# NoSuchThingAsRandom/EpidemicSimulator

Hardware: AMD Instinct MI355X
Metric: citizen-timesteps/sec (higher is better)
Workload: dtype u32 citizen word; u32 uniform vs ceil(q*2^32) (reference: f64 uniform; tolerance 2^-32 per draw); 1 GPU; uk64m: 64000000 citizens, 290000 Output Areas, 10 seeds, steps 1..667 of 5000, interventions on; seed=1592598545

## Files before the change

### epidemicsimulator_amd/csrc/esim_kernels_chunk.h

```cpp
#pragma once
#define BF_WIN 1024
__device__ __forceinline__ void block_scan_1024(uint32_t *v, uint32_t *wtmp)
{
    const uint32_t tid = threadIdx.x, lane = tid & 63u, wv = tid >> 6;
    uint32_t x = v[tid];
#pragma unroll
    for (int o = 1; o < 64; o <<= 1) { const uint32_t y = __shfl_up(x, o, 64); if (lane >= (uint32_t)o) x += y; }
    if (lane == 63u) wtmp[wv] = x;
    __syncthreads();
    if (tid == 0) { uint32_t a = 0; for (uint32_t w = 0; w < FIN_TPB / 64; ++w) { const uint32_t y = wtmp[w]; wtmp[w] = a; a += y; } }
    __syncthreads();
    v[tid] = x + wtmp[wv];
    __syncthreads();
}

__device__ __forceinline__ void future_body(const Dev &d, uint32_t max_ahead, uint32_t limit_t, uint32_t *win, uint32_t *wtmp)
{
    Ctrl *ctrl = d.ctrl;
    const uint32_t t0 = ld(&ctrl->t), tid = threadIdx.x;
    const uint32_t n_ahead = t0 > limit_t ? 0u : (limit_t - t0 + 1u < max_ahead ? limit_t - t0 + 1u : max_ahead);
    const int et = (int)d.exposed_time, it = (int)d.infected_time;
    const int base_idx = (int)(t0 + TE_BIAS) - et - 1 - it;
    { const int k = base_idx + (int)tid; win[tid] = (k >= 0 && k < (int)TE_SLOTS) ? ld(&d.hist[k]) : 0u; }
    __syncthreads();
// ... 926 lines not shown
}

struct ChunkShared {
    Decision dec[FREE_MAX];
    uint64_t thr[512];
};
struct RouteShared {
    uint32_t s_key[CHUNK_ROUTE_MAX];
    uint16_t s_bus[CHUNK_ROUTE_MAX];
    uint8_t s_inf[CHUNK_ROUTE_MAX];
    uint32_t s_cnt[CHUNK_ROUTE_MAX + 1];
};
#define SLOT_STEPS 4u
struct WaveScratch { uint32_t rounds; uint32_t cnt[FREE_MAX]; uint32_t sch[FREE_MAX]; uint32_t mem_id[64]; uint32_t mem_w[64]; uint4 desc[2u * (FREE_MAX / SLOT_STEPS + 1u)]; };

__device__ __forceinline__ void member_pairs(const Dev &d, Ctrl *ctrl, const ChunkShared &sm, WaveScratch &ws, const uint32_t *idx,
                                             uint32_t lo, uint32_t p_lo, uint32_t p_hi, uint32_t lane, uint32_t kind, uint32_t S, uint32_t t0 WORK_ARG,
                                             bool have_pre = false, uint32_t pre_m = 0u, uint32_t pre_w = 0u, uint32_t pre_base = 0u)
{
    const uint64_t seed = ((uint64_t)d.seed_hi << 32) | d.seed_lo;
    const uint32_t m_first = p_lo / S, m_last = (p_hi - 1u) / S;
    for (uint32_t mb = m_first; mb <= m_last; mb += 64u) {
        __builtin_amdgcn_wave_barrier();
        if (mb + lane <= m_last) {
            WORK_ADD(WK_MEMBERS, 1); WORK_ADD(WK_MEMBERS_IDX, idx ? 1 : 0);
            if (have_pre && mb == pre_base) { ws.mem_id[lane] = pre_m; ws.mem_w[lane] = pre_w; }
            else {
                const uint32_t m = idx ? idx[lo + mb + lane] : lo + mb + lane;
                ws.mem_id[lane] = m;
                ws.mem_w[lane] = d.cit[m];
            }
        }
        __builtin_amdgcn_wave_barrier();
        const uint32_t q_lo = max(p_lo, mb * S), q_hi = min(p_hi, (mb + 64u) * S);
#ifdef ESIM_WAVE_PROFILE
        if (lane == 0) ws.rounds += (q_hi - q_lo + 63u) / 64u;
#endif
        for (uint32_t p = q_lo + lane; p < q_hi; p += 64u) {
            const uint32_t um = p / S, si = p - um * S;
            const uint32_t m = ws.mem_id[um - mb], w = ws.mem_w[um - mb];
            const uint32_t te = CW_TE(w);
            WORK_ADD(WK_PAIRS, 1);
            if (te >= TE_RECOVERED && te != TE_SUSCEPTIBLE) continue;
            const uint4 dsc = ws.desc[2u * si];
            const uint32_t cnt23 = ws.desc[2u * si + 1u].x;
            const int jb = (int)(dsc.x & 127u) - 3;
            const uint32_t mk = (dsc.x >> 8) & 15u, atw = (dsc.x >> 12) & 15u, everywhere = (dsc.x >> 16) & 15u;
            const uint32_t vrel = CW_VAX_REL(w);
            const int js = (int)te + (((w & ~CW_KEEP) & ((1u << CW_TE_SHIFT) - 1u)) ? 1 : 0) - (int)(t0 + TE_BIAS);
            const int lim = min(js, vrel == CW_VAX_NONE ? (int)FREE_MAX : (int)vrel + 1) - jb;
            const uint32_t early = lim <= 0 ? 0u : lim >= (int)SLOT_STEPS ? 15u : (1u << lim) - 1u;
            const bool same = w & FL_SAME_AREA;
            const uint32_t here = kind == 0u ? (((w & FL_HAS_WORK) && !same) ? ~atw : 15u) : (same ? 15u : atw);
            const uint32_t act = mk & early & here;
            if (!act) continue;
            WORK_ADD(WK_PAIRS_ACTIVE, 1);
            const uint32_t nn = kind == 2u ? dsc.z : dsc.y;
            const uint32_t row = (w & FL_MASK_COMPLIANT) ? 0u : everywhere;
            uint64_t thr[SLOT_STEPS];
#pragma unroll
            for (uint32_t h = 0; h < SLOT_STEPS; ++h) thr[h] = sm.thr[(((row >> h) & 1u) << 8) + ((nn >> (8u * h)) & 255u)];
            const uint32_t gid = d.id_base + m;
            const uint32_t s_blk = (uint32_t)((int)t0 + jb) + (uint32_t)__builtin_ctz(act);
            uint32_t hit = 0u;
            if (kind == 2u) {
                const uint32_t cnt[SLOT_STEPS] = { dsc.w & 0xFFFFu, dsc.w >> 16, cnt23 & 0xFFFFu, cnt23 >> 16 };
                uint32_t kmax = 0u;
#pragma unroll
                for (uint32_t h = 0; h < SLOT_STEPS; ++h) if ((act >> h) & 1u) kmax = max(kmax, cnt[h]);
                const uint32_t first_act = act & (0u - act);
#ifdef ESIM_COUNT_WORK
                for (uint32_t h = 0; h < SLOT_STEPS; ++h) if ((act >> h) & 1u) WORK_ADD(WK_DRAWS, cnt[h]);
#endif
                for (uint32_t k = 0; k < kmax && !(hit & first_act); ++k) {
                    WORK_ADD(WK_BLOCKS, 1);
                    const philox_out o = esim_draw_block(seed, gid, s_blk, ESIM_SLOT_ROOM0 + k);
                    const uint32_t wd[SLOT_STEPS] = { o.w0, o.w1, o.w2, o.w3 };
#pragma unroll
                    for (uint32_t h = 0; h < SLOT_STEPS; ++h) if (((act >> h) & 1u) && k < cnt[h] && (uint64_t)wd[h] < thr[h]) hit |= 1u << h;
                }
            } else {
                WORK_ADD(WK_BLOCKS, 1); WORK_ADD(WK_DRAWS, __popc(act));
                const philox_out o = esim_draw_block(seed, gid, s_blk, kind == 0u ? ESIM_SLOT_HOME : ESIM_SLOT_WORK);
                const uint32_t wd[SLOT_STEPS] = { o.w0, o.w1, o.w2, o.w3 };
#pragma unroll
                for (uint32_t h = 0; h < SLOT_STEPS; ++h) if ((uint64_t)wd[h] < thr[h]) hit |= 1u << h;
                hit &= act;
            }
            if (hit) { WORK_ADD(WK_HITS, 1); expose_min(d, ctrl, m, w, (uint32_t)((int)t0 + jb) + (uint32_t)__builtin_ctz(hit), 0u); }
        }
    }
}

__device__ __forceinline__ uint32_t m96_nibble(const M96 &m, int p)
{
    if (p < 0) return (uint32_t)(m.lo << (-p)) & 15u;
    if (p >= 64) return p >= 96 ? 0u : (m.hi >> (p - 64)) & 15u;
    return (uint32_t)((m.lo >> p) | (p > 60 ? (unsigned long long)m.hi << (64 - p) : 0ull)) & 15u;
}

__device__ __forceinline__ uint32_t item_steps_regs(uint32_t c0, uint32_t c1, uint32_t lane, WaveScratch &ws, uint32_t t0, const M96 &AW, const M96 &EV)
{
    ws.cnt[lane] = c0;
    if (lane < FREE_MAX - 64u) ws.cnt[64u + lane] = c1;
// ... 28 lines not shown
__device__ __forceinline__ uint32_t fetch_slot(const Dev &d, uint32_t slot, uint32_t lane);
__device__ __forceinline__ void item_counts(const Dev &d, uint32_t x, uint32_t slot, uint32_t lane, uint32_t n, const M96 &AW,
                                            const M96 &BUS, uint32_t &c0, uint32_t &c1);
__device__ __forceinline__ void school_counts(const Dev &d, uint32_t s_sch, uint32_t lane, uint32_t n, const Decision &q0, const Decision &q1, WaveScratch &ws)
{
    uint32_t c0 = 0u, c1 = 0u;
    if (s_sch != 0xFFFFFFFFu) {
        if (lane < n) c0 = d.vec[(size_t)s_sch * FREE_MAX + lane];
        if (64u + lane < n) c1 = d.vec[(size_t)s_sch * FREE_MAX + 64u + lane];
    }
    ws.sch[lane] = c0;
    if (lane < FREE_MAX - 64u) ws.sch[64u + lane] = c1;
}

struct UnitSrc { uint32_t slot, link, own; };
__device__ __forceinline__ void list_or_units(const Dev &d, Ctrl *ctrl, const ChunkShared &sm, WaveScratch &ws, const uint32_t *idx,
                                              uint32_t lo, uint32_t hi, const UnitSrc &src, uint32_t lane, uint32_t kind, uint32_t S, uint32_t t0 WORK_ARG,
                                              bool have_pre = false, uint32_t pre_m = 0u, uint32_t pre_w = 0u)
{
    const uint32_t pairs = (hi - lo) * S;
    if (pairs == 0) return;
    if (pairs <= UNIT_INLINE) { member_pairs(d, ctrl, sm, ws, idx, lo, 0u, pairs, lane, kind, S, t0 WORK_PASS, have_pre, pre_m, pre_w); return; }
    const uint32_t n_units = (pairs + UNIT_PAIRS - 1u) / UNIT_PAIRS;
    const uint32_t r = ((blockIdx.x * TPB + threadIdx.x) >> 6) & (SUBQ - 1u);
    uint32_t start = 0;
    if (lane == 0) start = atomicAdd(&d.hot[(HOT_UNITS + r) * HOT_STRIDE], n_units);
    start = __shfl(start, 0, 64);
    UnitRec *q = d.units + (size_t)r * d.unit_qcap;
    if (start + n_units > d.unit_qcap) {
        for (uint32_t i = lane; i < n_units && start + i < d.unit_qcap; i += 64u) q[start + i].code = UNIT_NOOP;
        member_pairs(d, ctrl, sm, ws, idx, lo, 0u, pairs, lane, kind, S, t0 WORK_PASS, have_pre, pre_m, pre_w);
        return;
    }
    for (uint32_t i = lane; i < n_units; i += 64u) {
        const uint32_t p_lo = i * UNIT_PAIRS;
        q[start + i] = UnitRec{ src.slot, kind == 2u ? src.link : 0xFFFFFFFFu, lo, hi - lo, (kind << 30) | p_lo, src.own, p_lo / S, 0u };
    }
}

struct ItemFetch { uint32_t slot, id, a_lo, a_hi, b_lo, b_hi, aux, link, c0, c1; };
__device__ __forceinline__ uint32_t fetch_item(const Dev &d, uint32_t v, uint32_t lane)
{
    uint32_t x = 0u;
    if (lane < 8u) x = reinterpret_cast<const uint32_t *>(d.item_rec)[(size_t)v * 8u + lane];
    else if (lane == LANE_HSLOT) x = d.hitems[v];
    return x;
// ... 36 lines not shown
    if (f.slot < d.hcap) {
        item_counts(d, x, f.slot, lane, n, AW, BUS, f.c0, f.c1);
        iv_count(FX(x, 7), lane, AW, BUS, f.c0, f.c1);
    }
    return f;
}

__device__ __forceinline__ bool item_ok(const Dev &d, const ItemFetch &it)
{
    if (it.slot >= d.hcap) return false;
    if (it.id < d.n_bld) return it.a_lo <= it.a_hi && it.a_hi <= d.n && it.b_lo <= it.b_hi && it.b_hi <= d.n_wrk_idx;
    if (it.id < d.n_bld + d.n_room) return it.a_lo <= it.a_hi && it.a_hi <= d.n_room_idx && (it.link == 0xFFFFFFFFu || it.link < d.hcap);
    return true;
}
#define PAIR_SPREAD 1237u
__device__ __forceinline__ void route_pair_small(const Dev &d, Ctrl *ctrl, const ChunkShared &sm, uint32_t off, uint32_t sz, uint32_t j, uint32_t t0, uint32_t lane WORK_ARG)
{
    const uint64_t seed = ((uint64_t)d.seed_hi << 32) | d.seed_lo;
    const uint32_t s = t0 + j, mask = sm.dec[j].mask;
    uint32_t c = 0, w = 0, key = 0;
    bool inf = false;
    WORK_ADD(WK_ROUTE_PAIRS, lane == 0 ? 1 : 0); WORK_ADD(WK_RIDERS, lane < sz ? 1 : 0);
    bool can = false;
    if (lane < sz) {
        c = d.route_riders[off + lane];
        w = d.cit[c];
        inf = status_in_chunk(d, w, t0, j) == ESIM_INFECTED;
        const uint32_t te = CW_TE(w);
        can = !(w <= CW_MAKE(s + TE_BIAS, CW_BUS_EXPOSED | (w & CW_KEEP)) || (te >= TE_RECOVERED && te != TE_SUSCEPTIBLE) || j > CW_VAX_REL(w));
    }
    if (!__any(inf) || !__any(can)) return;
    uint32_t rank = 0;
    if (sz > d.bus_capacity) {
        if (lane < sz) key = philox4x32_10(d.id_base + c, s, ESIM_SLOT_BUS_ORDER, 0u, d.seed_lo, d.seed_hi).w0;
        for (uint32_t i = 0; i < sz; ++i) {
            const uint32_t ki = (uint32_t)__builtin_amdgcn_readlane((int)key, (int)i);
            rank += ki < key || (ki == key && i < lane);
        }
    }
    const uint32_t bus = rank / d.bus_capacity;
    const unsigned long long inf_m = __ballot(inf);
    uint32_t k = 0;
    const uint32_t n_bus = (sz + d.bus_capacity - 1u) / d.bus_capacity;
    for (uint32_t b = 0; b < n_bus; ++b) {
        const unsigned long long on_b = __ballot(lane < sz && bus == b);
        if (bus == b) k = (uint32_t)__popcll(on_b & inf_m);
    }
    if (lane < sz && k && can) {
        const uint32_t row = (!(w & FL_MASK_COMPLIANT) && mask == ESIM_MASK_EVERYWHERE) ? 1u : 0u;
        WORK_ADD(WK_BUS_DRAWS, 1);
        if (esim_u32(seed, d.id_base + c, s, ESIM_SLOT_BUS) < sm.thr[row * 256u + (k & 255u)]) { WORK_ADD(WK_HITS, 1); expose_min(d, ctrl, c, w, s, CW_BUS_EXPOSED); }
    }
}

template <uint32_t NT>
__device__ __forceinline__ void route_pair_big(const Dev &d, Ctrl *ctrl, const ChunkShared &sm, RouteShared &rs, uint32_t code, uint32_t t0, uint32_t n WORK_ARG)
{
    const uint64_t seed = ((uint64_t)d.seed_hi << 32) | d.seed_lo;
    const uint32_t r = code >> 7, j = code & 127u;
    if (r >= d.n_routes || j >= n) { if (threadIdx.x == 0) ctrl->error = (uint32_t)(-ESIM_ERANGE); return; }
    const uint32_t off = d.route_off[r], sz = d.route_off[r + 1] - off;
    if (sz > CHUNK_ROUTE_MAX) { if (threadIdx.x == 0) ctrl->error = (uint32_t)(-ESIM_ERANGE); return; }
    const uint32_t s = t0 + j, mask = sm.dec[j].mask;
    WORK_ADD(WK_ROUTE_PAIRS, threadIdx.x == 0 ? 1 : 0);
    int loc_inf = 0, loc_can = 0;
    for (uint32_t i = threadIdx.x; i < sz; i += NT) {
        const uint32_t c = d.route_riders[off + i];
// ... 19 lines not shown
    }
    __syncthreads();
    for (uint32_t i = threadIdx.x; i < sz; i += NT) {
        const uint32_t k = rs.s_cnt[rs.s_bus[i]];
        if (!k) continue;
        const uint32_t c = d.route_riders[off + i];
        const uint32_t w = d.cit[c], te = CW_TE(w);
        if (w <= CW_MAKE(s + TE_BIAS, CW_BUS_EXPOSED | (w & CW_KEEP)) || (te >= TE_RECOVERED && te != TE_SUSCEPTIBLE) || j > CW_VAX_REL(w)) continue;
        const uint32_t row = (!(w & FL_MASK_COMPLIANT) && mask == ESIM_MASK_EVERYWHERE) ? 1u : 0u;
        WORK_ADD(WK_BUS_DRAWS, 1);
        if (esim_u32(seed, d.id_base + c, s, ESIM_SLOT_BUS) < sm.thr[row * 256u + (k & 255u)]) { WORK_ADD(WK_HITS, 1); expose_min(d, ctrl, c, w, s, CW_BUS_EXPOSED); }
    }
    __syncthreads();
}

__global__ __launch_bounds__(TPB) void k_chunk_draw(Dev d, uint32_t n_mw)
{
    __shared__ ChunkShared sm;
    __shared__ WaveScratch wsc[TPB / 64];
    Ctrl *ctrl = d.ctrl;
    const uint32_t t0 = ctrl->chunk_t0, n = ctrl->chunk_ok;
    if (!ctrl->chunk_parallel || n == 0u) return;
    const uint32_t lane = threadIdx.x & 63u;
    const uint32_t wave = (blockIdx.x * TPB + threadIdx.x) >> 6, n_waves = (gridDim.x * TPB) >> 6;
    const uint32_t pt0 = PROF_NOW();
    WORK_TALLY;
    uint32_t p_items = 0u, p_item_max = 0u;
    const uint32_t per_wave = ld(&ctrl->items_per_wave);
    if ((unsigned long long)per_wave * n_mw > d.items_cap || n_waves % n_mw != 0u) return;
    const uint32_t G = n_waves / n_mw;
    const uint32_t T = d.used_pref[n_mw];
    const uint32_t coarse = d.used_pref[min(64u * lane, n_mw)];
    const uint32_t Tq = T / n_waves, Tr = T % n_waves;
    const uint32_t d_lo = Tq * wave + (uint32_t)(((unsigned long long)Tr * wave) / n_waves), d_hi = Tq * (wave + 1u) + (uint32_t)(((unsigned long long)Tr * (wave + 1u)) / n_waves);
// ... 20 lines not shown
    uint32_t code_l = 0u, off_l = 0u, sz_l = 0u;
    bool have = false;
    {
        const uint32_t k = lane * G + w_rep;
        if (k < K) {
            const uint32_t src = (w_base + n_mw - (uint32_t)(((unsigned long long)k * PAIR_SPREAD) % n_mw)) % n_mw;
            code_l = d.route_pairs[(size_t)src * K + k];
            have = k < d.pair_cnt[src] && (code_l >> 7) < d.n_routes && (code_l & 127u) < n;
        }
    }
    for (uint32_t i = threadIdx.x; i < n; i += TPB) sm.dec[i] = d.dec[i];
    for (uint32_t i = threadIdx.x; i < 512u; i += TPB) sm.thr[i] = d.thr[i];
    __syncthreads();
    const uint32_t route_base = d.n_bld + d.n_room;
    WaveScratch &ws = wsc[threadIdx.x >> 6];
    const Decision q0 = lane < n ? sm.dec[lane] : Decision{ 0u, 0u, 0u, 0u };
    const Decision q1 = 64u + lane < n ? sm.dec[64u + lane] : Decision{ 0u, 0u, 0u, 0u };
    M96 AW, BUS;
    schedule_masks(lane, n, q0, q1, AW, BUS);
    const M96 EV = { __ballot(lane < n && q0.mask == ESIM_MASK_EVERYWHERE), (uint32_t)__ballot(64u + lane < n && q1.mask == ESIM_MASK_EVERYWHERE) };
    if (d_lo < d_hi) sl_cur = fetch_slot(d, FX(id_cur, LANE_HSLOT), lane);
    if (have) { const uint32_t r = code_l >> 7; off_l = d.route_off[r]; sz_l = d.route_off[r + 1] - off_l; }
#ifdef ESIM_WAVE_PROFILE
    if (lane == 0) ws.rounds = 0u;
#endif
    uint32_t pst[5] = { 0u, 0u, 0u, 0u, 0u };
    const uint32_t pt1 = PROF_NOW();
    for (uint32_t v = d_lo; v < d_hi; ++v) {
        const uint32_t x = merge_fetch(id_cur, sl_cur, lane);
        id_cur = id_nxt;
// ... 8 lines not shown
        pst[0] += pi0 - pq0;
        (void)pi0; ++p_items; WORK_ADD(WK_ITEMS, lane == 0 ? 1 : 0);
        if (it.id < d.n_bld) {
            if (it.aux == ESIM_SCHOOL) continue;
            const uint32_t n_res = it.a_hi - it.a_lo, n_wrk = it.b_hi - it.b_lo;
            uint32_t rm = 0u, wm = 0u, rw = 0u, ww = 0u;
            if (lane < n_res) rm = d.res_idx ? d.res_idx[it.a_lo + lane] : it.a_lo + lane;
            if (lane < n_wrk) wm = d.wrk_idx[it.b_lo + lane];
            if (lane < n_res) rw = d.cit[rm];
            if (lane < n_wrk) ww = d.cit[wm];
            const uint32_t pq1 = PROF_NOW();
            const uint32_t S = item_steps_regs(it.c0, it.c1, lane, ws, t0, AW, EV);
            __builtin_amdgcn_wave_barrier();
            const uint32_t pq2 = PROF_NOW();
            const UnitSrc src = { it.slot, it.link, FX(x, 7) };
            list_or_units(d, ctrl, sm, ws, d.res_idx, it.a_lo, it.a_hi, src, lane, 0u, S, t0 WORK_PASS, true, rm, rw);
            const uint32_t pq3 = PROF_NOW();
            list_or_units(d, ctrl, sm, ws, d.wrk_idx, it.b_lo, it.b_hi, src, lane, 1u, S, t0 WORK_PASS, true, wm, ww);
            const uint32_t pq4 = PROF_NOW();
            pst[1] += pq1 - pi0; pst[2] += pq2 - pq1; pst[3] += pq3 - pq2; pst[4] += pq4 - pq3;
        } else {
            const uint32_t n_mem = it.a_hi - it.a_lo;
            uint32_t mm = 0u, mw = 0u;
            if (lane < n_mem) mm = d.room_idx[it.a_lo + lane];
            school_counts(d, it.link, lane, n, q0, q1, ws);
            if (lane < n_mem) mw = d.cit[mm];
            const uint32_t S = item_steps_regs(it.c0, it.c1, lane, ws, t0, AW, EV);
            __builtin_amdgcn_wave_barrier();
            const UnitSrc src = { it.slot, it.link, FX(x, 7) };
            list_or_units(d, ctrl, sm, ws, d.room_idx, it.a_lo, it.a_hi, src, lane, 2u, S, t0 WORK_PASS, true, mm, mw);
        }
        __builtin_amdgcn_wave_barrier();
        { const uint32_t dt = PROF_NOW() - pi0; p_item_max = dt > p_item_max ? dt : p_item_max; }
    }
    const uint32_t pt2 = PROF_NOW();
    for (uint32_t k0 = 0; k0 * G < K; k0 += 64u) {
        if (k0) {
            const uint32_t kk = (k0 + lane) * G + w_rep;
            have = false;
            if (kk < K) {
                const uint32_t src = (w_base + n_mw - (uint32_t)(((unsigned long long)kk * PAIR_SPREAD) % n_mw)) % n_mw;
                code_l = d.route_pairs[(size_t)src * K + kk];
                have = kk < d.pair_cnt[src] && (code_l >> 7) < d.n_routes && (code_l & 127u) < n;
            }
            if (have) { const uint32_t r = code_l >> 7; off_l = d.route_off[r]; sz_l = d.route_off[r + 1] - off_l; }
        }
        unsigned long long todo = __ballot(have);
        while (todo) {
            const int src_lane = __ffsll((long long)todo) - 1;
            todo &= todo - 1ull;
            const uint32_t code = __shfl(code_l, src_lane, 64), off = __shfl(off_l, src_lane, 64), sz = __shfl(sz_l, src_lane, 64);
            route_pair_small(d, ctrl, sm, off, sz, code & 127u, t0, lane WORK_PASS);
        }
    }
    WORK_FLUSH(d);
    const uint32_t pt3 = PROF_NOW();
#ifndef ESIM_PROFILE_UNITS
    PROF_PUT(d, 0, pt0); PROF_PUT(d, 1, pt1); PROF_PUT(d, 2, pt2); PROF_PUT(d, 3, pt3);
    PROF_PUT(d, 4, p_items); PROF_PUT(d, 5, p_item_max); PROF_PUT(d, 6, wsc[threadIdx.x >> 6].rounds);
    PROF_PUT(d, 11, pst[0]); PROF_PUT(d, 12, pst[1]); PROF_PUT(d, 13, pst[2]); PROF_PUT(d, 14, pst[3]); PROF_PUT(d, 15, pst[4]);
#endif
    (void)pst;
    (void)pt0; (void)pt1; (void)pt2; (void)pt3; (void)p_items; (void)p_item_max;
}

__global__ __launch_bounds__(TPB) void k_chunk_units(Dev d)
{
    __shared__ ChunkShared sm;
    __shared__ WaveScratch wsc[TPB / 64];
// ... 2 lines not shown
    const uint32_t t0 = ctrl->chunk_t0, n = ctrl->chunk_ok;
    if (!ctrl->chunk_parallel || n == 0u) return;
    const uint32_t lane = threadIdx.x & 63u;
    const uint32_t wave = (blockIdx.x * TPB + threadIdx.x) >> 6, n_waves = (gridDim.x * TPB) >> 6;
    const uint32_t pu0 = PROF_NOW();
    WORK_TALLY;
    uint32_t pu_n = 0u, pu_max = 0u, pu_it = 0u;
    const uint32_t qr = wave & (SUBQ - 1u), first = wave / SUBQ, step = n_waves / SUBQ;
    const uint32_t n_units = step ? min(ld(&d.hot[(HOT_UNITS + qr) * HOT_STRIDE]), d.unit_qcap) : 0u;
    const uint32_t n_pairs = min(ld(&d.hot[HOT_BIGPAIRS * HOT_STRIDE]), d.big_pairs_cap);
    if (__syncthreads_or(first < n_units) == 0 && n_pairs == 0u) return;
    for (uint32_t i = threadIdx.x; i < n; i += TPB) sm.dec[i] = d.dec[i];
    for (uint32_t i = threadIdx.x; i < 512u; i += TPB) sm.thr[i] = d.thr[i];
    __syncthreads();
    WaveScratch &ws = wsc[threadIdx.x >> 6];
    const uint32_t *q_words = reinterpret_cast<const uint32_t *>(d.units + (size_t)qr * d.unit_qcap);
    const Decision q0 = lane < n ? sm.dec[lane] : Decision{ 0u, 0u, 0u, 0u };
    const Decision q1 = 64u + lane < n ? sm.dec[64u + lane] : Decision{ 0u, 0u, 0u, 0u };
    M96 AW, BUS;
    schedule_masks(lane, n, q0, q1, AW, BUS);
    const M96 EV = { __ballot(lane < n && q0.mask == ESIM_MASK_EVERYWHERE), (uint32_t)__ballot(64u + lane < n && q1.mask == ESIM_MASK_EVERYWHERE) };
    auto unit_words = [&](uint32_t q) -> uint32_t { return lane < 8u ? q_words[(size_t)q * 8u + lane] : 0u; };
    auto member_id = [&](uint32_t u) -> uint32_t {
        const uint32_t code = FX(u, 4), kind = code >> 30, lo = FX(u, 2), n_mem = FX(u, 3), mf = FX(u, 6);
        if (code == UNIT_NOOP || mf + lane >= n_mem) return 0u;
        const uint32_t *idx = kind == 2u ? d.room_idx : kind == 1u ? d.wrk_idx : d.res_idx;
        return idx ? idx[lo + mf + lane] : lo + mf + lane;
    };
    const uint32_t pu1 = PROF_NOW();
    uint32_t u_0 = 0xFFFFFFFFu, u_1 = 0xFFFFFFFFu;
// ... 15 lines not shown
        const uint32_t mw = (mf + lane < n_mem) ? d.cit[mid] : 0u;
        uint32_t c0, c1;
        item_counts(d, xs, slot, lane, n, AW, BUS, c0, c1);
        iv_count(own, lane, AW, BUS, c0, c1);
        if (kind == 2u) {
            uint32_t s0 = 0u, s1 = 0u;
            if (link != 0xFFFFFFFFu) item_counts(d, ys, link, lane, n, AW, BUS, s0, s1);
            ws.sch[lane] = s0;
            if (lane < FREE_MAX - 64u) ws.sch[64u + lane] = s1;
        }
        const uint32_t *idx = kind == 2u ? d.room_idx : kind == 1u ? d.wrk_idx : d.res_idx;
        const uint32_t S = item_steps_regs(c0, c1, lane, ws, t0, AW, EV);
        __builtin_amdgcn_wave_barrier();
        const uint32_t pairs = n_mem * S;
        WORK_ADD(WK_UNITS, lane == 0 ? 1 : 0);
        member_pairs(d, ctrl, sm, ws, idx, lo, p_lo, min(pairs, p_lo + UNIT_PAIRS), lane, kind, S, t0 WORK_PASS, true, mid, mw, mf);
        __builtin_amdgcn_wave_barrier();
        { const uint32_t dt = PROF_NOW() - pui; pu_max = dt > pu_max ? dt : pu_max; pu_it += (min(pairs, p_lo + UNIT_PAIRS) - p_lo + 63u) / 64u; }
    }
    const uint32_t pu2 = PROF_NOW();
    WORK_FLUSH(d);
#ifdef ESIM_PROFILE_UNITS
    PROF_PUT(d, 0, pu0); PROF_PUT(d, 1, pu1); PROF_PUT(d, 2, pu2); PROF_PUT(d, 4, pu_n); PROF_PUT(d, 5, pu_max); PROF_PUT(d, 7, pu_it);
#endif
    (void)pu0; (void)pu1; (void)pu2; (void)pu_n; (void)pu_max; (void)pu_it;
    for (uint32_t q = blockIdx.x; q < n_pairs; q += gridDim.x) route_pair_big<TPB>(d, ctrl, sm, rs, d.route_pairs_big[q], t0, n WORK_PASS);
    WORK_FLUSH(d);
}

__global__ __launch_bounds__(TPB) void k_chunk_count(Dev d)
{
// ... 336 lines not shown
```

### epidemicsimulator_amd/csrc/esim_kernels_common.h

```cpp
#pragma once
#include <hip/hip_runtime.h>
#include "../../include/esim.h"
#include "esim_device.h"
#include "philox.h"

#define TPB 256
#define FIN_TPB 1024

__device__ __forceinline__ uint32_t status_of(uint32_t te, uint32_t t, uint32_t et, uint32_t it)
{
    if (te == TE_SUSCEPTIBLE) return ESIM_SUSCEPTIBLE;
    if (te == TE_VACCINATED) return ESIM_VACCINATED;
    if (te == TE_RECOVERED) return ESIM_RECOVERED;
    uint32_t d = t + TE_BIAS - te;
    if (d <= et) return ESIM_EXPOSED;
    if (d <= et + 1u + it) return ESIM_INFECTED;
    return ESIM_RECOVERED;
}

__device__ __forceinline__ uint32_t ld(const uint32_t *p)
{
    return __hip_atomic_load(p, __ATOMIC_RELAXED, __HIP_MEMORY_SCOPE_AGENT);
}

// ... 77 lines not shown
       WK_RECORDS,
       WK_DIRECT,
       WK_FOLDED,
       WK_ITEMS,
       WK_MEMBERS,
       WK_MEMBERS_IDX,
       WK_PAIRS,
       WK_PAIRS_ACTIVE,
       WK_BLOCKS,
       WK_DRAWS,
       WK_UNITS,
       WK_ROUTE_PAIRS,
       WK_RIDERS,
       WK_BUS_DRAWS,
       WK_HITS,
       WK_N };
#define WORK_TALLY uint32_t wk_[WK_N]; for (int wk_i = 0; wk_i < WK_N; ++wk_i) wk_[wk_i] = 0u
#define WORK_ADD(i, x) (wk_[i] += (uint32_t)(x))
#define WORK_FLUSH(d) do { for (int wk_i = 0; wk_i < WK_N; ++wk_i) { uint32_t x_ = wk_[wk_i]; for (int o_ = 32; o_ > 0; o_ >>= 1) x_ += __shfl_xor(x_, o_, 64); \
        if ((threadIdx.x & 63u) == 0 && x_) atomicAdd(&(d).work_cnt[wk_i], (unsigned long long)x_); wk_[wk_i] = 0u; } } while (0)
#define WORK_ARG , uint32_t *wk_
#define WORK_PASS , wk_
#else
#define WORK_TALLY do { } while (0)
#define WORK_ADD(i, x) do { } while (0)
#define WORK_FLUSH(d) do { } while (0)
#define WORK_ARG
#define WORK_PASS
#endif
```

### epidemicsimulator_amd/csrc/esim_kernels_tiny.h

```cpp
#pragma once

#define TINY_E 64u
#define TINY_WAVES (FIN_TPB / 64u)
#define TINY_INLINE 256u
#define TINY_TASKS 512u
#define TINY_BUS 8u
#define TINY_BIG 512u
#define TINY_NONE 0xFFFFFFFFu
#define TINY_SYNC() do { __builtin_amdgcn_fence(__ATOMIC_RELEASE, "workgroup"); __syncthreads(); __builtin_amdgcn_fence(__ATOMIC_ACQUIRE, "agent"); } while (0)

struct TinyShared {
    uint32_t e_c[TINY_E], e_w[TINY_E], e_iv[TINY_E];
    __attribute__((aligned(16))) uint32_t e_key[TINY_E][4];
    uint32_t uniq[4u * TINY_E];
    uint32_t n_uniq, n_tasks, n_big;
    uint32_t task[TINY_TASKS][3];
    uint32_t big[TINY_BIG];
};
static_assert(TINY_BIG >= TINY_E * TINY_BUS, "k_chunk_tiny: every entry's route on every bus step the guard admits must fit big[]");

__device__ __forceinline__ void tiny_counts(const TinyShared &ts, uint32_t E, uint32_t key, uint32_t lane, const M96 &AW, const M96 &BUS,
                                            uint32_t &c0, uint32_t &c1)
{
    c0 = 0u; c1 = 0u;
    for (uint32_t e = 0; e < E; ++e) {
        const uint32_t iv = ts.e_iv[e];
        if (ts.e_key[e][0] == key) iv_count(iv, lane, AW, BUS, c0, c1);
        if (ts.e_key[e][1] == key || ts.e_key[e][2] == key) iv_count(iv | IV_AS_WORK, lane, AW, BUS, c0, c1);
    }
}

__device__ __forceinline__ void tiny_list(const Dev &d, Ctrl *ctrl, const ChunkShared &sm, WaveScratch &ws, const uint32_t *idx, uint32_t lo,
                                          uint32_t p_lo, uint32_t p_hi, uint32_t lane, uint32_t kind, uint32_t S, uint32_t t0 WORK_ARG)
{
    if (p_lo < p_hi) member_pairs(d, ctrl, sm, ws, idx, lo, p_lo, p_hi, lane, kind, S, t0 WORK_PASS);
}

__global__ __launch_bounds__(FIN_TPB) void k_chunk_tiny(Dev d, int do_first, int do_next, uint32_t max_ahead, uint32_t limit_t)
{
    __shared__ BooksShared bs;
    __shared__ ChunkShared sm;
    __shared__ TinyShared ts;
    __shared__ __align__(16) unsigned char pool[sizeof(WaveScratch) * TINY_WAVES > sizeof(RouteShared) ? sizeof(WaveScratch) * TINY_WAVES : sizeof(RouteShared)];
    WaveScratch *wsc = reinterpret_cast<WaveScratch *>(pool);
    RouteShared &rs = *reinterpret_cast<RouteShared *>(pool);
    Ctrl *ctrl = d.ctrl;
    const uint32_t tid = threadIdx.x, lane = tid & 63u, wv = tid >> 6;
    TINY_PROF(d, 0);
    if (do_first) {
        future_body(d, max_ahead, limit_t, bs.win, bs.wtmp);
// ... 71 lines not shown
        TINY_PROF(d, 4);
        if (tid < 4u * TINY_E) {
            const uint32_t key = (&ts.e_key[0][0])[tid];
            bool first = key != TINY_NONE;
            const uint32_t me = tid >> 2, mk = tid & 3u;
            for (uint32_t e = 0; e <= me && first; ++e) {
                const uint4 k4 = *reinterpret_cast<const uint4 *>(&ts.e_key[e][0]);
                const uint32_t upto = e < me ? 4u : mk;
                if ((upto > 0u && k4.x == key) || (upto > 1u && k4.y == key) || (upto > 2u && k4.z == key) || (upto > 3u && k4.w == key)) first = false;
            }
            if (first) { WORK_ADD(WK_KEYS, 1); ts.uniq[atomicAdd(&ts.n_uniq, 1u)] = key; }
        }
        __syncthreads();
        TINY_PROF(d, 5);
        WaveScratch &ws = wsc[wv];
        const uint32_t n_uniq = ts.n_uniq, route_base = d.n_bld + d.n_room;
        for (uint32_t u = wv; u < n_uniq; u += TINY_WAVES) {
            const uint32_t key = ts.uniq[u];
            if (key >= route_base) {
                const uint32_t r = key - route_base;
                if (r >= d.n_routes) { if (lane == 0) RAISE(ctrl, ESIM_ERANGE, ERR_AT_ROUTE_ITEM); continue; }
                M96 ride = { 0ull, 0u };
                for (uint32_t e = 0; e < E; ++e) if (ts.e_key[e][3] == key) { const uint32_t iv = ts.e_iv[e]; const M96 I = m96_range(iv & 127u, (iv >> 7) & 127u); ride.lo |= I.lo & BUS.lo; ride.hi |= I.hi & BUS.hi; }
                const uint32_t off = d.route_off[r], sz = d.route_off[r + 1u] - off;
                for (uint32_t half = 0; half < 2u; ++half)
                    for (unsigned long long m = half ? (unsigned long long)ride.hi : ride.lo; m; m &= m - 1ull) {
                        const uint32_t j = 64u * half + (uint32_t)__builtin_ctzll(m);
                        if (sz <= 64u) route_pair_small(d, ctrl, sm, off, sz, j, t0, lane WORK_PASS);
                        else if (lane == 0) { const uint32_t at = atomicAdd(&ts.n_big, 1u); if (at < TINY_BIG) ts.big[at] = (r << 7) | j; else RAISE(ctrl, ESIM_ERANGE, ERR_AT_BIGPAIRS); }
                    }
                continue;
            }
            uint32_t c0, c1;
            tiny_counts(ts, E, key, lane, AW, BUS, c0, c1);
            WORK_ADD(WK_ITEMS, lane == 0 ? 1 : 0);
            if (key < d.n_bld) {
                const BldRec b = d.bld8[key];
                if (b.type == ESIM_SCHOOL) continue;
                if (b.res_lo > b.res_hi || b.res_hi > d.n || b.wrk_lo > b.wrk_hi || b.wrk_hi > d.n_wrk_idx) { if (lane == 0) RAISE(ctrl, ESIM_ERANGE, ERR_AT_ITEM_CHECK); continue; }
                const uint32_t n_res = b.res_hi - b.res_lo, n_wrk = b.wrk_hi - b.wrk_lo;
                uint32_t rm = 0u, wm = 0u, rw = 0u, ww = 0u;
                if (lane < n_res) rm = d.res_idx ? d.res_idx[b.res_lo + lane] : b.res_lo + lane;
                if (lane < n_wrk) wm = d.wrk_idx[b.wrk_lo + lane];
                if (lane < n_res) rw = d.cit[rm];
                if (lane < n_wrk) ww = d.cit[wm];
                const uint32_t S = item_steps_regs(c0, c1, lane, ws, t0, AW, EV);
                __builtin_amdgcn_wave_barrier();
                const uint32_t pr = n_res * S, pw = n_wrk * S;
                if (pr && pr <= TINY_INLINE) member_pairs(d, ctrl, sm, ws, d.res_idx, b.res_lo, 0u, pr, lane, 0u, S, t0 WORK_PASS, true, rm, rw);
                else if (!pr) { }
                else {
                    const uint32_t nu = (pr + TINY_INLINE - 1u) / TINY_INLINE; uint32_t at = 0u; if (lane == 0) at = atomicAdd(&ts.n_tasks, nu); at = FX(at, 0);
                    const uint32_t fit = at >= TINY_TASKS ? 0u : min(nu, TINY_TASKS - at);
                    for (uint32_t q = lane; q < fit; q += 64u) { ts.task[at + q][0] = key; ts.task[at + q][1] = 0u; ts.task[at + q][2] = q * TINY_INLINE; }
                    if (fit < nu) tiny_list(d, ctrl, sm, ws, d.res_idx, b.res_lo, fit * TINY_INLINE, pr, lane, 0u, S, t0 WORK_PASS);
                }
                if (pw && pw <= TINY_INLINE) member_pairs(d, ctrl, sm, ws, d.wrk_idx, b.wrk_lo, 0u, pw, lane, 1u, S, t0 WORK_PASS, true, wm, ww);
                else if (!pw) { }
                else {
                    const uint32_t nu = (pw + TINY_INLINE - 1u) / TINY_INLINE; uint32_t at = 0u; if (lane == 0) at = atomicAdd(&ts.n_tasks, nu); at = FX(at, 0);
                    const uint32_t fit = at >= TINY_TASKS ? 0u : min(nu, TINY_TASKS - at);
                    for (uint32_t q = lane; q < fit; q += 64u) { ts.task[at + q][0] = key; ts.task[at + q][1] = 1u; ts.task[at + q][2] = q * TINY_INLINE; }
                    if (fit < nu) tiny_list(d, ctrl, sm, ws, d.wrk_idx, b.wrk_lo, fit * TINY_INLINE, pw, lane, 1u, S, t0 WORK_PASS);
                }
            } else {
                const uint32_t r = key - d.n_bld;
                const uint32_t a_lo = d.room_off[r], a_hi = d.room_off[r + 1u], sch = d.room_bld[r];
                if (a_lo > a_hi || a_hi > d.n_room_idx) { if (lane == 0) RAISE(ctrl, ESIM_ERANGE, ERR_AT_ITEM_CHECK); continue; }
                uint32_t s0, s1;
                tiny_counts(ts, E, sch, lane, AW, BUS, s0, s1);
                ws.sch[lane] = s0;
                if (lane < FREE_MAX - 64u) ws.sch[64u + lane] = s1;
                uint32_t mm = 0u, mw = 0u;
                if (lane < a_hi - a_lo) { mm = d.room_idx[a_lo + lane]; mw = d.cit[mm]; }
                const uint32_t S = item_steps_regs(c0, c1, lane, ws, t0, AW, EV);
                __builtin_amdgcn_wave_barrier();
                const uint32_t pm = (a_hi - a_lo) * S;
                if (pm && pm <= TINY_INLINE) member_pairs(d, ctrl, sm, ws, d.room_idx, a_lo, 0u, pm, lane, 2u, S, t0 WORK_PASS, true, mm, mw);
                else if (!pm) { }
                else {
                    const uint32_t nu = (pm + TINY_INLINE - 1u) / TINY_INLINE; uint32_t at = 0u; if (lane == 0) at = atomicAdd(&ts.n_tasks, nu); at = FX(at, 0);
                    const uint32_t fit = at >= TINY_TASKS ? 0u : min(nu, TINY_TASKS - at);
                    for (uint32_t q = lane; q < fit; q += 64u) { ts.task[at + q][0] = key; ts.task[at + q][1] = 2u; ts.task[at + q][2] = q * TINY_INLINE; }
                    if (fit < nu) tiny_list(d, ctrl, sm, ws, d.room_idx, a_lo, fit * TINY_INLINE, pm, lane, 2u, S, t0 WORK_PASS);
                }
            }
            __builtin_amdgcn_wave_barrier();
        }
        __syncthreads();
        TINY_PROF(d, 6);
        const uint32_t n_tasks = min(ts.n_tasks, TINY_TASKS);
        for (uint32_t q = wv; q < n_tasks; q += TINY_WAVES) {
            const uint32_t key = ts.task[q][0], kind = ts.task[q][1], p_lo = ts.task[q][2];
// ... 33 lines not shown
```

Baseline: 52120 billion citizen-timesteps/s.

## Compact sparse Philox draws into per-wave LDS queue before drawing

Philox draws in the chunk draw kernel are no longer issued inline per lane. They are packed into descriptors and appended through a ballot/popcount compaction into a per-wave LDS queue of 128 entries, which is drained 64 at a time so every lane does a useful draw. Room draws lose the early exit after the first hit and are emitted per k round, and bus draws share the same path. This targets the divergence cost of sparse active pairs, but adds LDS traffic and extra draws for rooms, and it also sets waves_per_eu(5) on the kernel.

```diff
diff --git a/epidemicsimulator_amd/csrc/esim_kernels_chunk.h b/epidemicsimulator_amd/csrc/esim_kernels_chunk.h
--- a/epidemicsimulator_amd/csrc/esim_kernels_chunk.h
+++ b/epidemicsimulator_amd/csrc/esim_kernels_chunk.h
@@ -964,11 +964,54 @@
 #define SLOT_STEPS 4u
 struct WaveScratch { uint32_t rounds; uint32_t cnt[FREE_MAX]; uint32_t sch[FREE_MAX]; uint32_t mem_id[64]; uint32_t mem_w[64]; uint4 desc[2u * (FREE_MAX / SLOT_STEPS + 1u)]; };
 
-__device__ __forceinline__ void member_pairs(const Dev &d, Ctrl *ctrl, const ChunkShared &sm, WaveScratch &ws, const uint32_t *idx,
+__device__ __forceinline__ uint4 draw_entry(uint32_t m, uint32_t w, uint32_t nn, uint32_t first3, uint32_t act, uint32_t row, uint32_t slot)
+{
+    return make_uint4(m, w, nn, first3 | (act << 7) | (row << 11) | (slot << 15));
+}
+__device__ __forceinline__ void draw_now(const Dev &d, Ctrl *ctrl, const ChunkShared &sm, const uint4 e, uint32_t t0 WORK_ARG)
+{
+    const uint64_t seed = ((uint64_t)d.seed_hi << 32) | d.seed_lo;
+    const uint32_t act = (e.w >> 7) & 15u, row = (e.w >> 11) & 15u, slot = e.w >> 15;
+    const uint32_t s0 = t0 + (e.w & 127u) - 3u;
+    WORK_ADD(WK_BLOCKS, slot == ESIM_SLOT_BUS ? 0 : 1);
+    const philox_out o = esim_draw_block(seed, d.id_base + e.x, s0, slot);
+    const uint32_t wd[SLOT_STEPS] = { o.w0, o.w1, o.w2, o.w3 };
+    uint32_t hit = 0u;
+#pragma unroll
+    for (uint32_t h = 0; h < SLOT_STEPS; ++h) if ((uint64_t)wd[h] < sm.thr[(((row >> h) & 1u) << 8) + ((e.z >> (8u * h)) & 255u)]) hit |= 1u << h;
+    hit &= act;
+    if (hit) { WORK_ADD(WK_HITS, 1); expose_min(d, ctrl, e.x, e.y, s0 + (uint32_t)__builtin_ctz(hit), slot == ESIM_SLOT_BUS ? CW_BUS_EXPOSED : 0u); }
+}
+
+#define QUEUE_CAP 128u
+struct DirectDraw { };
+struct WaveQueue { uint4 *e; uint32_t n; };
+__device__ __forceinline__ void queue_drain(const Dev &d, Ctrl *ctrl, const ChunkShared &sm, WaveQueue &q, uint32_t t0, uint32_t lane WORK_ARG)
+{
+    const uint32_t take = min(q.n, 64u);
+    q.n -= take;
+    __builtin_amdgcn_wave_barrier();
+    WORK_ADD(WK_DRAIN_ROUNDS, lane == 0 ? 1 : 0);
+    if (lane < take) { WORK_ADD(WK_DRAINED, 1); draw_now(d, ctrl, sm, q.e[q.n + lane], t0 WORK_PASS); }
+    __builtin_amdgcn_wave_barrier();
+}
+__device__ __forceinline__ void draw_emit(const Dev &d, Ctrl *ctrl, const ChunkShared &sm, DirectDraw &, bool live, const uint4 e, uint32_t t0, uint32_t lane WORK_ARG)
+{
+    if (live) draw_now(d, ctrl, sm, e, t0 WORK_PASS);
+}
+__device__ __forceinline__ void draw_emit(const Dev &d, Ctrl *ctrl, const ChunkShared &sm, WaveQueue &q, bool live, const uint4 e, uint32_t t0, uint32_t lane WORK_ARG)
+{
+    const unsigned long long m = __ballot(live);
+    if (live) { WORK_ADD(WK_QUEUED, 1); q.e[q.n + (uint32_t)__popcll(m & ((1ull << lane) - 1ull))] = e; }
+    q.n += (uint32_t)__popcll(m);
+    if (q.n >= 64u) queue_drain(d, ctrl, sm, q, t0, lane WORK_PASS);
+}
+
+template <class Q>
+__device__ __forceinline__ void member_pairs(const Dev &d, Ctrl *ctrl, const ChunkShared &sm, WaveScratch &ws, Q &q, const uint32_t *idx,
                                              uint32_t lo, uint32_t p_lo, uint32_t p_hi, uint32_t lane, uint32_t kind, uint32_t S, uint32_t t0 WORK_ARG,
                                              bool have_pre = false, uint32_t pre_m = 0u, uint32_t pre_w = 0u, uint32_t pre_base = 0u)
 {
-    const uint64_t seed = ((uint64_t)d.seed_hi << 32) | d.seed_lo;
     const uint32_t m_first = p_lo / S, m_last = (p_hi - 1u) / S;
     for (uint32_t mb = m_first; mb <= m_last; mb += 64u) {
         __builtin_amdgcn_wave_barrier();
@@ -986,58 +1029,44 @@
 #ifdef ESIM_WAVE_PROFILE
         if (lane == 0) ws.rounds += (q_hi - q_lo + 63u) / 64u;
 #endif
-        for (uint32_t p = q_lo + lane; p < q_hi; p += 64u) {
+        for (uint32_t pb = q_lo; pb < q_hi; pb += 64u) {
+            const uint32_t p = pb + lane;
             const uint32_t um = p / S, si = p - um * S;
-            const uint32_t m = ws.mem_id[um - mb], w = ws.mem_w[um - mb];
+            uint32_t m = 0u, w = 0u, act = 0u, nn = 0u, row = 0u, first3 = 0u, cnt01 = 0u, cnt23 = 0u;
+            if (p < q_hi) { m = ws.mem_id[um - mb]; w = ws.mem_w[um - mb]; WORK_ADD(WK_PAIRS, 1); }
             const uint32_t te = CW_TE(w);
-            WORK_ADD(WK_PAIRS, 1);
-            if (te >= TE_RECOVERED && te != TE_SUSCEPTIBLE) continue;
-            const uint4 dsc = ws.desc[2u * si];
-            const uint32_t cnt23 = ws.desc[2u * si + 1u].x;
-            const int jb = (int)(dsc.x & 127u) - 3;
-            const uint32_t mk = (dsc.x >> 8) & 15u, atw = (dsc.x >> 12) & 15u, everywhere = (dsc.x >> 16) & 15u;
-            const uint32_t vrel = CW_VAX_REL(w);
-            const int js = (int)te + (((w & ~CW_KEEP) & ((1u << CW_TE_SHIFT) - 1u)) ? 1 : 0) - (int)(t0 + TE_BIAS);
-            const int lim = min(js, vrel == CW_VAX_NONE ? (int)FREE_MAX : (int)vrel + 1) - jb;
-            const uint32_t early = lim <= 0 ? 0u : lim >= (int)SLOT_STEPS ? 15u : (1u << lim) - 1u;
-            const bool same = w & FL_SAME_AREA;
-            const uint32_t here = kind == 0u ? (((w & FL_HAS_WORK) && !same) ? ~atw : 15u) : (same ? 15u : atw);
-            const uint32_t act = mk & early & here;
-            if (!act) continue;
-            WORK_ADD(WK_PAIRS_ACTIVE, 1);
-            const uint32_t nn = kind == 2u ? dsc.z : dsc.y;
-            const uint32_t row = (w & FL_MASK_COMPLIANT) ? 0u : everywhere;
-            uint64_t thr[SLOT_STEPS];
-#pragma unroll
-            for (uint32_t h = 0; h < SLOT_STEPS; ++h) thr[h] = sm.thr[(((row >> h) & 1u) << 8) + ((nn >> (8u * h)) & 255u)];
-            const uint32_t gid = d.id_base + m;
-            const uint32_t s_blk = (uint32_t)((int)t0 + jb) + (uint32_t)__builtin_ctz(act);
-            uint32_t hit = 0u;
+            if (p < q_hi && !(te >= TE_RECOVERED && te != TE_SUSCEPTIBLE)) {
+                const uint4 dsc = ws.desc[2u * si];
+                const int jb = (int)(dsc.x & 127u) - 3;
+                const uint32_t mk = (dsc.x >> 8) & 15u, atw = (dsc.x >> 12) & 15u, everywhere = (dsc.x >> 16) & 15u;
+                const uint32_t vrel = CW_VAX_REL(w);
+                const int js = (int)te + (((w & ~CW_KEEP) & ((1u << CW_TE_SHIFT) - 1u)) ? 1 : 0) - (int)(t0 + TE_BIAS);
+                const int lim = min(js, vrel == CW_VAX_NONE ? (int)FREE_MAX : (int)vrel + 1) - jb;
+                const uint32_t early = lim <= 0 ? 0u : lim >= (int)SLOT_STEPS ? 15u : (1u << lim) - 1u;
+                const bool same = w & FL_SAME_AREA;
+                const uint32_t here = kind == 0u ? (((w & FL_HAS_WORK) && !same) ? ~atw : 15u) : (same ? 15u : atw);
+                act = mk & early & here;
+                first3 = dsc.x & 127u;
+                nn = kind == 2u ? dsc.z : dsc.y;
+                row = (w & FL_MASK_COMPLIANT) ? 0u : everywhere;
+                cnt01 = dsc.w;
+                if (kind == 2u) cnt23 = ws.desc[2u * si + 1u].x;
+                WORK_ADD(WK_PAIRS_ACTIVE, act ? 1 : 0);
+            }
             if (kind == 2u) {
-                const uint32_t cnt[SLOT_STEPS] = { dsc.w & 0xFFFFu, dsc.w >> 16, cnt23 & 0xFFFFu, cnt23 >> 16 };
-                uint32_t kmax = 0u;
-#pragma unroll
-                for (uint32_t h = 0; h < SLOT_STEPS; ++h) if ((act >> h) & 1u) kmax = max(kmax, cnt[h]);
-                const uint32_t first_act = act & (0u - act);
+                const uint32_t cnt[SLOT_STEPS] = { cnt01 & 0xFFFFu, cnt01 >> 16, cnt23 & 0xFFFFu, cnt23 >> 16 };
 #ifdef ESIM_COUNT_WORK
                 for (uint32_t h = 0; h < SLOT_STEPS; ++h) if ((act >> h) & 1u) WORK_ADD(WK_DRAWS, cnt[h]);
 #endif
-                for (uint32_t k = 0; k < kmax && !(hit & first_act); ++k) {
-                    WORK_ADD(WK_BLOCKS, 1);
-                    const philox_out o = esim_draw_block(seed, gid, s_blk, ESIM_SLOT_ROOM0 + k);
-                    const uint32_t wd[SLOT_STEPS] = { o.w0, o.w1, o.w2, o.w3 };
-#pragma unroll
-                    for (uint32_t h = 0; h < SLOT_STEPS; ++h) if (((act >> h) & 1u) && k < cnt[h] && (uint64_t)wd[h] < thr[h]) hit |= 1u << h;
+                for (uint32_t k = 0; ; ++k) {
+                    const uint32_t act_k = act & ((k < cnt[0] ? 1u : 0u) | (k < cnt[1] ? 2u : 0u) | (k < cnt[2] ? 4u : 0u) | (k < cnt[3] ? 8u : 0u));
+                    if (!__any(act_k != 0u)) break;
+                    draw_emit(d, ctrl, sm, q, act_k != 0u, draw_entry(m, w, nn, first3, act_k, row, ESIM_SLOT_ROOM0 + k), t0, lane WORK_PASS);
                 }
             } else {
-                WORK_ADD(WK_BLOCKS, 1); WORK_ADD(WK_DRAWS, __popc(act));
-                const philox_out o = esim_draw_block(seed, gid, s_blk, kind == 0u ? ESIM_SLOT_HOME : ESIM_SLOT_WORK);
-                const uint32_t wd[SLOT_STEPS] = { o.w0, o.w1, o.w2, o.w3 };
-#pragma unroll
-                for (uint32_t h = 0; h < SLOT_STEPS; ++h) if ((uint64_t)wd[h] < thr[h]) hit |= 1u << h;
-                hit &= act;
-            }
-            if (hit) { WORK_ADD(WK_HITS, 1); expose_min(d, ctrl, m, w, (uint32_t)((int)t0 + jb) + (uint32_t)__builtin_ctz(hit), 0u); }
+                WORK_ADD(WK_DRAWS, __popc(act));
+                draw_emit(d, ctrl, sm, q, act != 0u, draw_entry(m, w, nn, first3, act, row, kind == 0u ? ESIM_SLOT_HOME : ESIM_SLOT_WORK), t0, lane WORK_PASS);
+            }
         }
     }
 }
@@ -1096,13 +1125,13 @@
 }
 
 struct UnitSrc { uint32_t slot, link, own; };
-__device__ __forceinline__ void list_or_units(const Dev &d, Ctrl *ctrl, const ChunkShared &sm, WaveScratch &ws, const uint32_t *idx,
+__device__ __forceinline__ void list_or_units(const Dev &d, Ctrl *ctrl, const ChunkShared &sm, WaveScratch &ws, WaveQueue &dq, const uint32_t *idx,
                                               uint32_t lo, uint32_t hi, const UnitSrc &src, uint32_t lane, uint32_t kind, uint32_t S, uint32_t t0 WORK_ARG,
                                               bool have_pre = false, uint32_t pre_m = 0u, uint32_t pre_w = 0u)
 {
     const uint32_t pairs = (hi - lo) * S;
     if (pairs == 0) return;
-    if (pairs <= UNIT_INLINE) { member_pairs(d, ctrl, sm, ws, idx, lo, 0u, pairs, lane, kind, S, t0 WORK_PASS, have_pre, pre_m, pre_w); return; }
+    if (pairs <= UNIT_INLINE) { member_pairs(d, ctrl, sm, ws, dq, idx, lo, 0u, pairs, lane, kind, S, t0 WORK_PASS, have_pre, pre_m, pre_w); return; }
     const uint32_t n_units = (pairs + UNIT_PAIRS - 1u) / UNIT_PAIRS;
     const uint32_t r = ((blockIdx.x * TPB + threadIdx.x) >> 6) & (SUBQ - 1u);
     uint32_t start = 0;
@@ -1111,7 +1140,7 @@
     UnitRec *q = d.units + (size_t)r * d.unit_qcap;
     if (start + n_units > d.unit_qcap) {
         for (uint32_t i = lane; i < n_units && start + i < d.unit_qcap; i += 64u) q[start + i].code = UNIT_NOOP;
-        member_pairs(d, ctrl, sm, ws, idx, lo, 0u, pairs, lane, kind, S, t0 WORK_PASS, have_pre, pre_m, pre_w);
+        member_pairs(d, ctrl, sm, ws, dq, idx, lo, 0u, pairs, lane, kind, S, t0 WORK_PASS, have_pre, pre_m, pre_w);
         return;
     }
     for (uint32_t i = lane; i < n_units; i += 64u) {
@@ -1178,9 +1207,9 @@
     return true;
 }
 #define PAIR_SPREAD 1237u
-__device__ __forceinline__ void route_pair_small(const Dev &d, Ctrl *ctrl, const ChunkShared &sm, uint32_t off, uint32_t sz, uint32_t j, uint32_t t0, uint32_t lane WORK_ARG)
-{
-    const uint64_t seed = ((uint64_t)d.seed_hi << 32) | d.seed_lo;
+template <class Q>
+__device__ __forceinline__ void route_pair_small(const Dev &d, Ctrl *ctrl, const ChunkShared &sm, Q &q, uint32_t off, uint32_t sz, uint32_t j, uint32_t t0, uint32_t lane WORK_ARG)
+{
     const uint32_t s = t0 + j, mask = sm.dec[j].mask;
     uint32_t c = 0, w = 0, key = 0;
     bool inf = false;
@@ -1210,11 +1239,10 @@
         const unsigned long long on_b = __ballot(lane < sz && bus == b);
         if (bus == b) k = (uint32_t)__popcll(on_b & inf_m);
     }
-    if (lane < sz && k && can) {
-        const uint32_t row = (!(w & FL_MASK_COMPLIANT) && mask == ESIM_MASK_EVERYWHERE) ? 1u : 0u;
-        WORK_ADD(WK_BUS_DRAWS, 1);
-        if (esim_u32(seed, d.id_base + c, s, ESIM_SLOT_BUS) < sm.thr[row * 256u + (k & 255u)]) { WORK_ADD(WK_HITS, 1); expose_min(d, ctrl, c, w, s, CW_BUS_EXPOSED); }
-    }
+    const bool draw = lane < sz && k && can;
+    const uint32_t h = s & 3u, row = (!(w & FL_MASK_COMPLIANT) && mask == ESIM_MASK_EVERYWHERE) ? 1u : 0u;
+    WORK_ADD(WK_BUS_DRAWS, draw ? 1 : 0);
+    draw_emit(d, ctrl, sm, q, draw, draw_entry(c, w, (k & 255u) << (8u * h), (s & ~3u) + 3u - t0, 1u << h, row << h, ESIM_SLOT_BUS), t0, lane WORK_PASS);
 }
 
 template <uint32_t NT>
@@ -1264,10 +1292,11 @@
     __syncthreads();
 }
 
-__global__ __launch_bounds__(TPB) void k_chunk_draw(Dev d, uint32_t n_mw)
+__global__ __launch_bounds__(TPB) __attribute__((amdgpu_waves_per_eu(5))) void k_chunk_draw(Dev d, uint32_t n_mw)
 {
     __shared__ ChunkShared sm;
     __shared__ WaveScratch wsc[TPB / 64];
+    __shared__ uint4 queue[TPB / 64][QUEUE_CAP];
     Ctrl *ctrl = d.ctrl;
     const uint32_t t0 = ctrl->chunk_t0, n = ctrl->chunk_ok;
     if (!ctrl->chunk_parallel || n == 0u) return;
@@ -1318,6 +1347,7 @@
     __syncthreads();
     const uint32_t route_base = d.n_bld + d.n_room;
     WaveScratch &ws = wsc[threadIdx.x >> 6];
+    WaveQueue dq = { queue[threadIdx.x >> 6], 0u };
     const Decision q0 = lane < n ? sm.dec[lane] : Decision{ 0u, 0u, 0u, 0u };
     const Decision q1 = 64u + lane < n ? sm.dec[64u + lane] : Decision{ 0u, 0u, 0u, 0u };
     M96 AW, BUS;
@@ -1356,9 +1386,9 @@
             __builtin_amdgcn_wave_barrier();
             const uint32_t pq2 = PROF_NOW();
             const UnitSrc src = { it.slot, it.link, FX(x, 7) };
-            list_or_units(d, ctrl, sm, ws, d.res_idx, it.a_lo, it.a_hi, src, lane, 0u, S, t0 WORK_PASS, true, rm, rw);
+            list_or_units(d, ctrl, sm, ws, dq, d.res_idx, it.a_lo, it.a_hi, src, lane, 0u, S, t0 WORK_PASS, true, rm, rw);
             const uint32_t pq3 = PROF_NOW();
-            list_or_units(d, ctrl, sm, ws, d.wrk_idx, it.b_lo, it.b_hi, src, lane, 1u, S, t0 WORK_PASS, true, wm, ww);
+            list_or_units(d, ctrl, sm, ws, dq, d.wrk_idx, it.b_lo, it.b_hi, src, lane, 1u, S, t0 WORK_PASS, true, wm, ww);
             const uint32_t pq4 = PROF_NOW();
             pst[1] += pq1 - pi0; pst[2] += pq2 - pq1; pst[3] += pq3 - pq2; pst[4] += pq4 - pq3;
         } else {
@@ -1370,7 +1400,7 @@
             const uint32_t S = item_steps_regs(it.c0, it.c1, lane, ws, t0, AW, EV);
             __builtin_amdgcn_wave_barrier();
             const UnitSrc src = { it.slot, it.link, FX(x, 7) };
-            list_or_units(d, ctrl, sm, ws, d.room_idx, it.a_lo, it.a_hi, src, lane, 2u, S, t0 WORK_PASS, true, mm, mw);
+            list_or_units(d, ctrl, sm, ws, dq, d.room_idx, it.a_lo, it.a_hi, src, lane, 2u, S, t0 WORK_PASS, true, mm, mw);
         }
         __builtin_amdgcn_wave_barrier();
         { const uint32_t dt = PROF_NOW() - pi0; p_item_max = dt > p_item_max ? dt : p_item_max; }
@@ -1392,9 +1422,10 @@
             const int src_lane = __ffsll((long long)todo) - 1;
             todo &= todo - 1ull;
             const uint32_t code = __shfl(code_l, src_lane, 64), off = __shfl(off_l, src_lane, 64), sz = __shfl(sz_l, src_lane, 64);
-            route_pair_small(d, ctrl, sm, off, sz, code & 127u, t0, lane WORK_PASS);
-        }
-    }
+            route_pair_small(d, ctrl, sm, dq, off, sz, code & 127u, t0, lane WORK_PASS);
+        }
+    }
+    if (dq.n) queue_drain(d, ctrl, sm, dq, t0, lane WORK_PASS);
     WORK_FLUSH(d);
     const uint32_t pt3 = PROF_NOW();
 #ifndef ESIM_PROFILE_UNITS
@@ -1427,6 +1458,7 @@
     for (uint32_t i = threadIdx.x; i < 512u; i += TPB) sm.thr[i] = d.thr[i];
     __syncthreads();
     WaveScratch &ws = wsc[threadIdx.x >> 6];
+    DirectDraw direct;
     const uint32_t *q_words = reinterpret_cast<const uint32_t *>(d.units + (size_t)qr * d.unit_qcap);
     const Decision q0 = lane < n ? sm.dec[lane] : Decision{ 0u, 0u, 0u, 0u };
     const Decision q1 = 64u + lane < n ? sm.dec[64u + lane] : Decision{ 0u, 0u, 0u, 0u };
@@ -1472,7 +1504,7 @@
         __builtin_amdgcn_wave_barrier();
         const uint32_t pairs = n_mem * S;
         WORK_ADD(WK_UNITS, lane == 0 ? 1 : 0);
-        member_pairs(d, ctrl, sm, ws, idx, lo, p_lo, min(pairs, p_lo + UNIT_PAIRS), lane, kind, S, t0 WORK_PASS, true, mid, mw, mf);
+        member_pairs(d, ctrl, sm, ws, direct, idx, lo, p_lo, min(pairs, p_lo + UNIT_PAIRS), lane, kind, S, t0 WORK_PASS, true, mid, mw, mf);
         __builtin_amdgcn_wave_barrier();
         { const uint32_t dt = PROF_NOW() - pui; pu_max = dt > pu_max ? dt : pu_max; pu_it += (min(pairs, p_lo + UNIT_PAIRS) - p_lo + 63u) / 64u; }
     }
diff --git a/epidemicsimulator_amd/csrc/esim_kernels_common.h b/epidemicsimulator_amd/csrc/esim_kernels_common.h
--- a/epidemicsimulator_amd/csrc/esim_kernels_common.h
+++ b/epidemicsimulator_amd/csrc/esim_kernels_common.h
@@ -115,6 +115,9 @@
        WK_RIDERS,
        WK_BUS_DRAWS,
        WK_HITS,
+       WK_QUEUED,
+       WK_DRAINED,
+       WK_DRAIN_ROUNDS,
        WK_N };
 #define WORK_TALLY uint32_t wk_[WK_N]; for (int wk_i = 0; wk_i < WK_N; ++wk_i) wk_[wk_i] = 0u
 #define WORK_ADD(i, x) (wk_[i] += (uint32_t)(x))
diff --git a/epidemicsimulator_amd/csrc/esim_kernels_tiny.h b/epidemicsimulator_amd/csrc/esim_kernels_tiny.h
--- a/epidemicsimulator_amd/csrc/esim_kernels_tiny.h
+++ b/epidemicsimulator_amd/csrc/esim_kernels_tiny.h
@@ -33,7 +33,8 @@
 __device__ __forceinline__ void tiny_list(const Dev &d, Ctrl *ctrl, const ChunkShared &sm, WaveScratch &ws, const uint32_t *idx, uint32_t lo,
                                           uint32_t p_lo, uint32_t p_hi, uint32_t lane, uint32_t kind, uint32_t S, uint32_t t0 WORK_ARG)
 {
-    if (p_lo < p_hi) member_pairs(d, ctrl, sm, ws, idx, lo, p_lo, p_hi, lane, kind, S, t0 WORK_PASS);
+    DirectDraw direct;
+    if (p_lo < p_hi) member_pairs(d, ctrl, sm, ws, direct, idx, lo, p_lo, p_hi, lane, kind, S, t0 WORK_PASS);
 }
 
 __global__ __launch_bounds__(FIN_TPB) void k_chunk_tiny(Dev d, int do_first, int do_next, uint32_t max_ahead, uint32_t limit_t)
@@ -135,6 +136,7 @@
         __syncthreads();
         TINY_PROF(d, 5);
         WaveScratch &ws = wsc[wv];
+        DirectDraw direct;
         const uint32_t n_uniq = ts.n_uniq, route_base = d.n_bld + d.n_room;
         for (uint32_t u = wv; u < n_uniq; u += TINY_WAVES) {
             const uint32_t key = ts.uniq[u];
@@ -147,7 +149,7 @@
                 for (uint32_t half = 0; half < 2u; ++half)
                     for (unsigned long long m = half ? (unsigned long long)ride.hi : ride.lo; m; m &= m - 1ull) {
                         const uint32_t j = 64u * half + (uint32_t)__builtin_ctzll(m);
-                        if (sz <= 64u) route_pair_small(d, ctrl, sm, off, sz, j, t0, lane WORK_PASS);
+                        if (sz <= 64u) route_pair_small(d, ctrl, sm, direct, off, sz, j, t0, lane WORK_PASS);
                         else if (lane == 0) { const uint32_t at = atomicAdd(&ts.n_big, 1u); if (at < TINY_BIG) ts.big[at] = (r << 7) | j; else RAISE(ctrl, ESIM_ERANGE, ERR_AT_BIGPAIRS); }
                     }
                 continue;
@@ -168,7 +170,7 @@
                 const uint32_t S = item_steps_regs(c0, c1, lane, ws, t0, AW, EV);
                 __builtin_amdgcn_wave_barrier();
                 const uint32_t pr = n_res * S, pw = n_wrk * S;
-                if (pr && pr <= TINY_INLINE) member_pairs(d, ctrl, sm, ws, d.res_idx, b.res_lo, 0u, pr, lane, 0u, S, t0 WORK_PASS, true, rm, rw);
+                if (pr && pr <= TINY_INLINE) member_pairs(d, ctrl, sm, ws, direct, d.res_idx, b.res_lo, 0u, pr, lane, 0u, S, t0 WORK_PASS, true, rm, rw);
                 else if (!pr) { }
                 else {
                     const uint32_t nu = (pr + TINY_INLINE - 1u) / TINY_INLINE; uint32_t at = 0u; if (lane == 0) at = atomicAdd(&ts.n_tasks, nu); at = FX(at, 0);
@@ -176,7 +178,7 @@
                     for (uint32_t q = lane; q < fit; q += 64u) { ts.task[at + q][0] = key; ts.task[at + q][1] = 0u; ts.task[at + q][2] = q * TINY_INLINE; }
                     if (fit < nu) tiny_list(d, ctrl, sm, ws, d.res_idx, b.res_lo, fit * TINY_INLINE, pr, lane, 0u, S, t0 WORK_PASS);
                 }
-                if (pw && pw <= TINY_INLINE) member_pairs(d, ctrl, sm, ws, d.wrk_idx, b.wrk_lo, 0u, pw, lane, 1u, S, t0 WORK_PASS, true, wm, ww);
+                if (pw && pw <= TINY_INLINE) member_pairs(d, ctrl, sm, ws, direct, d.wrk_idx, b.wrk_lo, 0u, pw, lane, 1u, S, t0 WORK_PASS, true, wm, ww);
                 else if (!pw) { }
                 else {
                     const uint32_t nu = (pw + TINY_INLINE - 1u) / TINY_INLINE; uint32_t at = 0u; if (lane == 0) at = atomicAdd(&ts.n_tasks, nu); at = FX(at, 0);
@@ -197,7 +199,7 @@
                 const uint32_t S = item_steps_regs(c0, c1, lane, ws, t0, AW, EV);
                 __builtin_amdgcn_wave_barrier();
                 const uint32_t pm = (a_hi - a_lo) * S;
-                if (pm && pm <= TINY_INLINE) member_pairs(d, ctrl, sm, ws, d.room_idx, a_lo, 0u, pm, lane, 2u, S, t0 WORK_PASS, true, mm, mw);
+                if (pm && pm <= TINY_INLINE) member_pairs(d, ctrl, sm, ws, direct, d.room_idx, a_lo, 0u, pm, lane, 2u, S, t0 WORK_PASS, true, mm, mw);
                 else if (!pm) { }
                 else {
                     const uint32_t nu = (pm + TINY_INLINE - 1u) / TINY_INLINE; uint32_t at = 0u; if (lane == 0) at = atomicAdd(&ts.n_tasks, nu); at = FX(at, 0);
```

After: 51760 billion citizen-timesteps/s. Within noise of the previous version (-0.7%).
